# aikiriao/LINNE

Hardware: AMD Instinct MI355X
Metric: frames/sec encode (-m 7) + decode, 44.1 kHz stereo, bit-exact; 1/2/4/8 GPU (higher is better)
Workload: dtype f64; 1 GPU; encode -m 7: 1 x 60 min 44.1 kHz int16 2-channel per GPU = 15504 frames of 10240 samples (tail 9280), MS on, PCM resident in HBM; decode = inverse hot path on the encode output; frames_per_gpu=15504, channels=2, preset=7, tracks_per_gpu=1

## Files before the change

linne_amd/csrc/lnn_k_autocorr.h:

```cpp
#ifndef LNN_K_AUTOCORR_H_INCLUDED
#define LNN_K_AUTOCORR_H_INCLUDED

__device__ __forceinline__ const DevClass &job_class(const Plan &p, uint32_t job) { return p.cls[p.cls_of_frame[(job / p.R) / p.C]]; }
__device__ __forceinline__ double q1_stale_first_trial(const Plan &p, uint32_t job, const DevClass &c)
{
    const uint32_t f = (job / p.R) / p.C, mid = c.na >> 1;
    if (mid >= c.n) return 0.0;
    const size_t i = ((size_t)p.frame_map[f] * p.C + (p.C - 1u)) * p.S + mid;
    return ((double)pcm_at(p, i) * p.scale) * p.sintab[c.sin_off + mid];
}

template <int P> struct AcCfg {
    static constexpr int K = 5;
    static constexpr int NT = (P >= 128) ? 8 : ((P >= 64) ? 7 : (P >= 32) ? 6 : (P >= 16) ? 5 : (P >= 8) ? 4 : (P >= 4) ? 3 : 2);
    static constexpr int T = (P >= 32) ? 60 : 20;
    static constexpr int lanes(int t) { return ((P >> t) + 1 + K - 1) / K; }
    static constexpr int halo(int t) { return K * lanes(t) + K; }
    static constexpr int rb(int t) { return ((T + halo(t) + 3 + 4 * K - 1) / (4 * K)) * (4 * K); }
    static constexpr int lpj() { int s = 0; for (int t = 0; t < NT; t++) s += lanes(t); return s; }
    static constexpr int ringsum() { int s = 0; for (int t = 0; t < NT; t++) s += rb(t); return s; }
    static constexpr int maxpad() { int m = 0; for (int t = 0; t < NT; t++) { const int p = P >> t, z = p > 4 ? p : 4, v = (1 << t) * z; if (v > m) m = v; } return m; }
    static constexpr int LPJ = lpj();
    static constexpr int JPW = 64 / LPJ;
    static constexpr int NS = JPW * NT;
// ... 239 lines not shown
__device__ __forceinline__ void autocorr_lane(const Plan &p, uint32_t layer, uint32_t cur, uint32_t q_end, uint32_t job, uint32_t t, bool active)
{
    constexpr int U = 4;
    constexpr uint32_t np = K - 1;
    const DevClass &c = job_class(p, job);
    const uint32_t u = 1u << t;
    const uint32_t n = active ? (c.na / u) : 1u;
    const uint32_t upl = n + (np > 4 ? np : 4);
    const double *wt = p.wtab + (active ? c.wt_off[layer][t] : 0u);
    const int32_t *xi = p.xint + (size_t)(job / p.R) * p.S;
    const double *xd = p.sig + ((size_t)job * 2 + cur) * p.S;
    double stale = 0.0;
    if (active && (n & 1u) && u == 1u) stale = q1_stale_first_trial(p, job, c);
    else if (active && (n & 1u)) {
        const uint32_t m = n >> 1, n2 = 2 * n, si = (u / 2 - 1) * n2 + m;
        const double xv = L0 ? ((double)xi[si] * p.scale) : xd[si];
        stale = xv * (c.trial_div[layer][t - 1] * (double)m * (double)(n2 - 1 - m));
    }
    const bool odd = (n & 1u) != 0;
    const uint32_t mid = n >> 1;
    uint32_t g_loc = 0, g_ubase = 0, g_left = active ? u : 0u;
    auto gen_issue = [&](double &rx, double &rw, uint32_t &rloc) {
        const bool in_unit = (g_loc < n) && (g_left != 0);
        rx = L0 ? ((double)xi[in_unit ? (g_ubase + g_loc) : 0u] * p.scale) : xd[in_unit ? (g_ubase + g_loc) : 0u];
        rw = wt[g_loc];
        rloc = in_unit ? g_loc : 0xFFFFFFFFu;
        const bool wrap = (g_loc + 1 >= upl);
        g_loc = wrap ? 0u : g_loc + 1;
        g_ubase = (wrap && g_left > 1) ? g_ubase + n : g_ubase;
        g_left = (wrap && g_left) ? g_left - 1 : g_left;
    };
    auto gen_finish = [&](double rx, double rw, uint32_t rloc) -> double {
        const double v = rx * rw;
        const double vv = (odd && rloc == mid) ? stale : v;
        return (rloc == 0xFFFFFFFFu) ? 0.0 : vv;
    };
    double r[K], w[K + U], fx[D][U], fw[D][U]; uint32_t fl[D][U];
#pragma unroll
    for (int j = 0; j < K; j++) {
        r[j] = 0.0;
        double rx, rw; uint32_t rl;
        gen_issue(rx, rw, rl);
        w[j] = gen_finish(rx, rw, rl);
    }
#pragma unroll
    for (int d = 0; d < D; d++) {
#pragma unroll
        for (int j = 0; j < U; j++) gen_issue(fx[d][j], fw[d][j], fl[d][j]);
    }
    uint32_t a_unit = 0, flush_pos = n;
    double *out = p.acorr + ((size_t)job * LNN_MAXT + t) * LNN_ACW;
#pragma unroll 1
    for (uint32_t q0 = 0; q0 < q_end; q0 += U * D) {
#pragma unroll
        for (int d = 0; d < D; d++) {
            if (active && q0 + (uint32_t)(d * U) >= flush_pos) {
                double *o = out + (size_t)a_unit * K;
#pragma unroll
                for (int j = 0; j < K; j++) { o[j] = r[j]; r[j] = 0.0; }
                a_unit++;
                flush_pos = (a_unit < u) ? (flush_pos + upl) : 0xFFFFFFFFu;
            }
#pragma unroll
            for (int j = 0; j < U; j++) w[K + j] = gen_finish(fx[d][j], fw[d][j], fl[d][j]);
#pragma unroll
            for (int j = 0; j < U; j++) gen_issue(fx[d][j], fw[d][j], fl[d][j]);
#pragma unroll
            for (int tt = 0; tt < U; tt++) {
#pragma unroll
                for (int j = 0; j < K; j++) r[j] += w[tt] * w[tt + j];
            }
#pragma unroll
            for (int j = 0; j < K; j++) w[j] = w[j + U];
        }
    }
}

#define ACS_T 32
template <int K, int J0, int JN, bool L0, int NT>
__device__ __forceinline__ void autocorr_shared(const Plan &p, uint32_t layer, uint32_t cur, uint32_t row0, uint32_t nrows, uint32_t rstride,
        uint32_t na, uint32_t wt_off, uint32_t t, uint32_t wave, uint32_t lane, double (*tile)[ACS_T][65])
{
    constexpr uint32_t np = K - 1, pad = (np > 4 ? np : 4);
    constexpr int L = ((int)np + 3) / 4 * 4;
    constexpr int NSLOT = (ACS_T + NT - 1) / NT;
    const uint32_t u = 1u << t, n = na / u, upl = n + pad, ntiles = na / ACS_T;
    const double *wt = p.wtab + wt_off;
    uint32_t myrow = row0 + lane; if (myrow >= nrows) myrow = nrows - 1;
    const bool store = (row0 + lane) < nrows;
    double *out = p.acorr + ((size_t)myrow * rstride * LNN_MAXT + t) * LNN_ACW;
    double preA[NSLOT], preB[NSLOT], wA = 0.0, wB = 0.0, wcur = 0.0;
    const uint32_t ls = lane & (ACS_T - 1u), lr = lane / ACS_T;
    constexpr uint32_t RPS = 64 / ACS_T;
    auto issue = [&](uint32_t tile_idx, double *pre, double &wv) {
#pragma unroll
        for (int i = 0; i < NSLOT; i++) {
            const uint32_t k = wave + (uint32_t)i * NT;
            if (k < 64 / RPS) {
                uint32_t r = row0 + RPS * k + lr; if (r >= nrows) r = nrows - 1;
                const uint32_t sidx = tile_idx * ACS_T + ls;
                if (L0) pre[i] = (double)p.xint[(size_t)r * p.S + sidx] * p.scale;
                else pre[i] = p.sig[((size_t)r * 2 + cur) * p.S + sidx];
            }
        }
        wv = wt[(tile_idx * ACS_T + ls) % n];
    };
    auto commit = [&](uint32_t buf, const double *pre, double wv) {
#pragma unroll
        for (int i = 0; i < NSLOT; i++) {
            const uint32_t k = wave + (uint32_t)i * NT;
            if (k < 64 / RPS) tile[buf][ls][RPS * k + lr] = pre[i];
        }
        wcur = wv;
    };
    auto lane_bcast = [&](double v, uint32_t src_lane) -> double {
        const int lo = __builtin_amdgcn_readlane(__double2loint(v), (int)src_lane), hi = __builtin_amdgcn_readlane(__double2hiint(v), (int)src_lane);
        return __hiloint2double(hi, lo);
    };
    issue(0, preA, wA); commit(0, preA, wA);
    __syncthreads();
    if (ntiles > 1) issue(1, preB, wB);
    if (ntiles > 2) issue(2, preA, wA);
    uint32_t g_loc = 0, g_tile = 0, g_off = 0;
    struct D4 { double v0, v1, v2, v3; };
    auto next4 = [&]() -> D4 {
        D4 d; d.v0 = 0.0; d.v1 = 0.0; d.v2 = 0.0; d.v3 = 0.0;
        if (g_loc < n && g_tile < ntiles) {
            const double *src = &tile[g_tile & 1u][g_off][lane];
            d.v0 = src[0] * lane_bcast(wcur, g_off); d.v1 = src[65] * lane_bcast(wcur, g_off + 1);
            d.v2 = src[130] * lane_bcast(wcur, g_off + 2); d.v3 = src[195] * lane_bcast(wcur, g_off + 3);
            g_off += 4;
            if (g_off == ACS_T) {
                g_off = 0; g_tile++;
                if (g_tile < ntiles) {
                    if (g_tile & 1u) { commit(1, preB, wB); __syncthreads(); if (g_tile + 2 < ntiles) issue(g_tile + 2, preB, wB); }
                    else             { commit(0, preA, wA); __syncthreads(); if (g_tile + 2 < ntiles) issue(g_tile + 2, preA, wA); }
                }
            }
        }
        g_loc += 4; if (g_loc >= upl) g_loc = 0;
        return d;
    };
    constexpr int W = L + 4, NG = W / 4;
    double r[JN], w[W];
#pragma unroll
    for (int j = 0; j < JN; j++) r[j] = 0.0;
#pragma unroll
    for (int j = 0; j < L / 4; j++) { const D4 d = next4(); w[4 * j] = d.v0; w[4 * j + 1] = d.v1; w[4 * j + 2] = d.v2; w[4 * j + 3] = d.v3; }
    uint32_t a_unit = 0, flush_pos = n, q0 = 0;
    bool done = false;
#pragma unroll 1
    while (!done) {
#pragma unroll
        for (int g = 0; g < NG; g++) {
            if (!done) {
                if (q0 >= flush_pos) {
                    if (store) {
                        double *o = out + (size_t)a_unit * K + J0;
#pragma unroll
                        for (int j = 0; j < JN; j++) o[j] = r[j];
                    }
#pragma unroll
                    for (int j = 0; j < JN; j++) r[j] = 0.0;
                    a_unit++;
                    flush_pos += upl;
                    done = (a_unit == u);
                }
                if (!done) {
                    const D4 d = next4();
                    w[(4 * g + L) % W] = d.v0; w[(4 * g + L + 1) % W] = d.v1; w[(4 * g + L + 2) % W] = d.v2; w[(4 * g + L + 3) % W] = d.v3;
#pragma unroll
                    for (int tt = 0; tt < 4; tt++) {
#pragma unroll
                        for (int j = 0; j < JN; j++) r[j] += w[(4 * g + tt) % W] * w[(4 * g + tt + J0 + j) % W];
                    }
                    q0 += 4;
                }
            }
        }
    }
}

template <int P, bool L0, int TT, int J0, int JN, int NW, int T = 32>
__device__ __forceinline__ void autocorr_rows(const Plan &p, uint32_t layer, uint32_t cur, uint32_t row0, uint32_t nrows, uint32_t rstride,
        uint32_t na, const DevClass &c0, uint32_t wave, uint32_t lane, double (*xt)[T][65], double (*wtile)[32])
{
    constexpr int NT = AcCfg<P>::NT, NLD = L0 ? T / 4 : T / 2, PT = P >> TT;
    constexpr int NSLOT = (NLD + NW - 1) / NW;
    constexpr int TU = (PT > T) ? PT / T : 1;
    constexpr uint32_t RPI = L0 ? 256u / T : 128u / T, LPR = 64u / RPI;
    static_assert((T == 32 || T == 16) && PT <= 32 && (TU * T) % PT == 0 && J0 + JN <= PT + 1, "register rings: sample m lives in slot m % PT, and the tile loop is unrolled over TU * T samples");
    typedef typename std::conditional<L0, int4, lnn_d2>::type XV;
    const uint32_t ntiles = na / T, seg = na >> (NT - 1), nt = na >> TT;
    uint32_t myrow = row0 + lane; if (myrow >= nrows) myrow = nrows - 1;
    const bool store = (row0 + lane) < nrows;
    double *out = p.acorr + ((size_t)myrow * rstride * LNN_MAXT + TT) * LNN_ACW + J0;
    const uint32_t lrow = lane / LPR, lsmp = (L0 ? 4u : 2u) * (lane % LPR);
    const void *src[NSLOT];
#pragma unroll
    for (int i = 0; i < NSLOT; i++) {
        const uint32_t k = wave + (uint32_t)i * NW;
        uint32_t r = row0 + RPI * (k < (uint32_t)NLD ? k : 0u) + lrow; if (r >= nrows) r = nrows - 1;
        if (L0) src[i] = p.xint + (size_t)r * p.S + lsmp;
        else src[i] = p.sig + ((size_t)r * 2 + cur) * p.S + lsmp;
    }
    const double *wt = p.wtab + (uint32_t)__builtin_amdgcn_readfirstlane((int)c0.wt_off[layer][TT]);
    const double *wts = p.wtab + (uint32_t)__builtin_amdgcn_readfirstlane((int)c0.wt_off[layer][wave < (uint32_t)NT ? wave : 0u]);
    const uint32_t wnt = na >> (wave < (uint32_t)NT ? wave : 0u);
    uint32_t wloc = 0;
    (void)wt; (void)nt;
    XV pre[NSLOT]; double prew = 0.0;
    auto issue = [&](uint32_t tile_idx) {
#pragma unroll
        for (int i = 0; i < NSLOT; i++)
            if (wave + (uint32_t)i * NW < (uint32_t)NLD) pre[i] = *(const XV *)((L0 ? (const char *)src[i] + (size_t)tile_idx * T * 4 : (const char *)src[i] + (size_t)tile_idx * T * 8));
        if (wave < (uint32_t)NT) {
            uint32_t l = wloc + (lane & (T - 1u)); if (l >= wnt) l -= wnt;
            prew = wts[l];
            wloc += T; if (wloc >= wnt) wloc -= wnt;
        }
    };
    auto commit = [&](uint32_t buf) {
#pragma unroll
        for (int i = 0; i < NSLOT; i++) {
            const uint32_t k = wave + (uint32_t)i * NW;
            if (k < (uint32_t)NLD) {
                const uint32_t r = RPI * k + lrow;
                if (L0) {
                    const int4 v = *(const int4 *)&pre[i];
                    xt[buf][lsmp][r] = (double)v.x * p.scale; xt[buf][lsmp + 1][r] = (double)v.y * p.scale;
                    xt[buf][lsmp + 2][r] = (double)v.z * p.scale; xt[buf][lsmp + 3][r] = (double)v.w * p.scale;
                } else { const lnn_d2 v = *(const lnn_d2 *)&pre[i]; xt[buf][lsmp][r] = v.x; xt[buf][lsmp + 1][r] = v.y; }
            }
        }
        if (wave < (uint32_t)NT && lane < T) wtile[buf * NT + wave][lane] = prew;
    };
    double r[JN], ring[PT], q[JN];
#pragma unroll
    for (int j = 0; j < JN; j++) { r[j] = 0.0; q[j] = 0.0; }
#pragma unroll
    for (int j = 0; j < PT; j++) ring[j] = 0.0;
    auto read_group = [&](uint32_t slot, double *xv, double *wv) {
        const uint32_t buf = slot / T, o = slot % T;
#pragma unroll
        for (int i = 0; i < 4; i++) xv[i] = xt[buf][o + i][lane];
        const lnn_d2 a = *(const lnn_d2 *)&wtile[buf * NT + TT][o], b = *(const lnn_d2 *)&wtile[buf * NT + TT][o + 2];
        wv[0] = a.x; wv[1] = a.y; wv[2] = b.x; wv[3] = b.y;
    };
    issue(0); commit(0);
    __syncthreads();
    double xv[4], wv[4], vcur;
    read_group(0, xv, wv);
    vcur = xv[0] * wv[0];
    uint32_t to_b = seg, bcount = 0, unit = 0;
#pragma unroll 1
    for (uint32_t t0 = 0; t0 < ntiles; t0 += TU) {
#pragma unroll
      for (int h = 0; h < TU; h++) {
        const uint32_t ti = t0 + (uint32_t)h, buf = ti & 1u;
        if (ti + 1 < ntiles) issue(ti + 1);
#pragma unroll
        for (int g = 0; g < T / 4; g++) {
            if (g == T / 4 - 1) {
                if (ti + 1 < ntiles) commit(buf ^ 1u);
                __syncthreads();
            }
            double nx[4], nw[4];
            read_group((buf * T + 4 * (uint32_t)g + 4) % (2 * T), nx, nw);
#pragma unroll
            for (int i = 0; i < 4; i++) {
#pragma unroll
                for (int j = 0; j < JN; j++) r[j] += q[j];
                const double v = vcur;
#pragma unroll
                for (int j = 0; j < JN; j++) q[j] = (J0 + j == 0) ? (v * v) : (ring[((h * T + 4 * g + i - (J0 + j)) % PT + PT) % PT] * v);
                ring[(h * T + 4 * g + i) % PT] = v;
                vcur = (i < 3) ? (xv[(i + 1) & 3] * wv[(i + 1) & 3]) : (nx[0] * nw[0]);
            }
#pragma unroll
            for (int i = 0; i < 4; i++) { xv[i] = nx[i]; wv[i] = nw[i]; }
            to_b -= 4;
            if (to_b == 0) {
                to_b = seg; bcount++;
                if ((bcount & ((1u << (NT - 1 - TT)) - 1u)) == 0) {
#pragma unroll
                    for (int j = 0; j < JN; j++) { r[j] += q[j]; q[j] = 0.0; }
                    if (store) {
                        double *o = out + (size_t)unit * (PT + 1);
#pragma unroll
                        for (int j = 0; j < JN; j++) o[j] = r[j];
                    }
#pragma unroll
                    for (int j = 0; j < JN; j++) r[j] = 0.0;
#pragma unroll
                    for (int j = 0; j < PT; j++) ring[j] = 0.0;
                    unit++;
                }
            }
        }
      }
    }
}

template <int P> struct AcsWaves;
template <> struct AcsWaves<16> { static constexpr int NW = 8; };
template <> struct AcsWaves<8>  { static constexpr int NW = 5; };
template <> struct AcsWaves<4>  { static constexpr int NW = 10; };
template <> struct AcsWaves<2>  { static constexpr int NW = 5; };

#define ACS_ROWS(P_) ((P_) <= 4 || p.rows16)
template <int P, bool L0>
__global__ __launch_bounds__(64 * AcsWaves<P>::NW, (P >= 8) ? 4 : 5) void k_autocorr_lane(Plan p, uint32_t layer, uint32_t cur, uint32_t na_max)
{
    using Cfg = AcCfg<P>;
    constexpr int NT = Cfg::NT, NW = AcsWaves<P>::NW;
    __shared__ double tile[2][ACS_T][65];
    __shared__ __attribute__((aligned(16))) double wts_mem[2 * NT * 32];
    const uint32_t wave = threadIdx.x >> 6, lane = threadIdx.x & 63u;
    const uint32_t rstride = L0 ? p.R : 1u;
    const RowRuns &rr = p.runs[L0 ? 0 : 1];
    const uint32_t b = gridDim.x - 1u - blockIdx.x;
    uint32_t run = 0;
    while (run + 1 < rr.n && b >= rr.blk_begin[run + 1]) run++;
    const uint32_t row0 = rr.row_begin[run] + (b - rr.blk_begin[run]) * 64u, nrows = rr.row_begin[run + 1];
    uint32_t row = row0 + lane;
    const bool inrange = row < nrows;
    if (!inrange) row = nrows - 1;
    const uint32_t job = row * rstride;
    const uint32_t ci = p.cls_of_frame[(job / p.R) / p.C];
    const uint32_t ci0 = (uint32_t)__builtin_amdgcn_readfirstlane((int)ci);
    const DevClass &c0 = p.cls[ci0];
    const uint32_t na = (uint32_t)__builtin_amdgcn_readfirstlane((int)c0.na);
    const bool fast = __all(ci == ci0) && c0.ntrials[layer] == (uint32_t)NT && (na % (4u << (NT - 1))) == 0 && (na % ACS_T) == 0;
    constexpr int NWS = (P == 4) ? 3 : (P == 2) ? 2 : NW;
#define ACS_RUN(T_, K_, J0_, JN_) autocorr_shared<K_, J0_, JN_, L0, NWS>(p, layer, cur, row0, nrows, rstride, na, \
        (uint32_t)__builtin_amdgcn_readfirstlane((int)c0.wt_off[layer][T_]), T_, wave, lane, tile)
    if constexpr (P <= 16) {
        if (fast && (na >> (NT - 1)) >= 32u && (p.S & 3u) == 0 && ACS_ROWS(P)) {
            double (*wtile)[32] = (double (*)[32])wts_mem;
#define ROWS_RUN(T_, J0_, JN_) autocorr_rows<P, L0, T_, J0_, JN_, NW>(p, layer, cur, row0, nrows, rstride, na, c0, wave, lane, tile, wtile)
            if constexpr (P == 16) switch (wave) {
                case 0: ROWS_RUN(0, 10, 7); break; case 1: ROWS_RUN(0, 0, 5); break; case 2: ROWS_RUN(0, 5, 5); break; case 3: ROWS_RUN(1, 0, 5); break;
                case 4: ROWS_RUN(4, 0, 2); break;  case 5: ROWS_RUN(1, 5, 4); break; case 6: ROWS_RUN(2, 0, 5); break; default: ROWS_RUN(3, 0, 3); break;
            } else if constexpr (P == 8) switch (wave) {
                case 0: ROWS_RUN(0, 0, 5); break; case 1: ROWS_RUN(0, 5, 4); break; case 2: ROWS_RUN(1, 0, 5); break; case 3: ROWS_RUN(2, 0, 3); break;
                default: ROWS_RUN(3, 0, 2); break;
            } else if constexpr (P == 4) switch (wave) {
                case 0: ROWS_RUN(0, 0, 1); break; case 1: ROWS_RUN(0, 1, 1); break; case 2: ROWS_RUN(0, 2, 1); break; case 3: ROWS_RUN(0, 3, 1); break;
                case 4: ROWS_RUN(0, 4, 1); break; case 5: ROWS_RUN(1, 0, 1); break; case 6: ROWS_RUN(1, 1, 1); break; case 7: ROWS_RUN(1, 2, 1); break;
                case 8: ROWS_RUN(2, 0, 1); break; default: ROWS_RUN(2, 1, 1); break;
            } else switch (wave) {
                case 0: ROWS_RUN(0, 0, 1); break; case 1: ROWS_RUN(0, 1, 1); break; case 2: ROWS_RUN(0, 2, 1); break;
                case 3: ROWS_RUN(1, 0, 1); break; default: ROWS_RUN(1, 1, 1); break;
            }
#undef ROWS_RUN
            return;
        }
    }
    if (fast) {
        if (P == 16) switch (wave) {
            case 0: ACS_RUN(0, 17, 10, 7); break; case 1: ACS_RUN(0, 17, 0, 5); break;  case 2: ACS_RUN(0, 17, 5, 5); break;
            case 3: ACS_RUN(1, 9, 0, 5); break;   case 4: ACS_RUN(4, 2, 0, 2); break;   case 5: ACS_RUN(1, 9, 5, 4); break;
            case 6: ACS_RUN(2, 5, 0, 5); break;   default: ACS_RUN(3, 3, 0, 3); break;
        } else if (P == 8) switch (wave) {
            case 0: ACS_RUN(0, 9, 0, 5); break;   case 1: ACS_RUN(0, 9, 5, 4); break;   case 2: ACS_RUN(1, 5, 0, 5); break;
            case 3: ACS_RUN(2, 3, 0, 3); break;   default: ACS_RUN(3, 2, 0, 2); break;
        } else if (P == 4) switch (wave) {
            case 0: ACS_RUN(0, 5, 0, 5); break;   case 1: ACS_RUN(1, 3, 0, 3); break;   case 2: ACS_RUN(2, 2, 0, 2); break;   default: break;
        } else switch (wave) {
            case 0: ACS_RUN(0, 3, 0, 3); break;   case 1: ACS_RUN(1, 2, 0, 2); break;   default: break;
        }
        return;
    }
#undef ACS_RUN
    if (wave >= (uint32_t)NT) return;
    const uint32_t t = wave;
    const bool active = inrange && (t < job_class(p, job).ntrials[layer]);
    constexpr int D = 1;
    const uint32_t q_end = na_max + Cfg::MAXPAD + 8 + 4 * D;
    switch (P >> t) {
    case 16: if (P >= 16) autocorr_lane<17, L0, D>(p, layer, cur, q_end, job, t, active); break;
    case 8:  if (P >= 8)  autocorr_lane<9, L0, D>(p, layer, cur, q_end, job, t, active); break;
    case 4:  if (P >= 4)  autocorr_lane<5, L0, D>(p, layer, cur, q_end, job, t, active); break;
    case 2:  autocorr_lane<3, L0, D>(p, layer, cur, q_end, job, t, active); break;
    default: autocorr_lane<2, L0, D>(p, layer, cur, q_end, job, t, active); break;
    }
}

template <int P> static void launch_autocorr_small(hipStream_t st, const Plan &p, uint32_t layer, uint32_t cur, uint32_t na_max)
{
    const RowRuns &rr = p.runs[layer == 0 ? 0 : 1];
    const dim3 grid(rr.blk_begin[rr.n]);
    if (layer == 0) hipLaunchKernelGGL((k_autocorr_lane<P, true>), grid, dim3(64 * AcsWaves<P>::NW), 0, st, p, layer, cur, na_max);
    else hipLaunchKernelGGL((k_autocorr_lane<P, false>), grid, dim3(64 * AcsWaves<P>::NW), 0, st, p, layer, cur, na_max);
}

template <int P> struct ApCfg {
    static constexpr int NT = (P >= 16) ? 5 : (P >= 8) ? 4 : (P >= 4) ? 3 : 2;
    static constexpr int nch() { int s = 0; for (int t = 0; t < NT; t++) s += (P >> t) + 1; return s; }
    static constexpr int NCH = nch();
    static constexpr int CHUNK = (P >= 16) ? 128 : (P >= 8) ? 128 : 256;
    static constexpr int trial_of(int ch) { int t = 0; while (ch >= (P >> t) + 1) { ch -= (P >> t) + 1; t++; } return t; }
    static constexpr int lag_of(int ch) { int t = 0; while (ch >= (P >> t) + 1) { ch -= (P >> t) + 1; t++; } return ch; }
};
template <int P, bool L0, int NTH>
__global__ __launch_bounds__(NTH) void k_autocorr_prod(Plan p, uint32_t layer, uint32_t cur)
{
    using Cfg = ApCfg<P>;
    constexpr int NT = Cfg::NT, NCH = Cfg::NCH, CHUNK = Cfg::CHUNK, NPROD = NTH - 64;
    static_assert(NCH <= 64, "one wave adds up all chains");
    __shared__ double sv[2][NT][CHUNK + P];
    __shared__ uint32_t srem[2][NT][CHUNK + P];
    __shared__ __attribute__((aligned(16))) double sprod[2][NCH][CHUNK + 2];
    const uint32_t row = blockIdx.x, tid = threadIdx.x, job = L0 ? row * p.R : row;
    const DevClass &c = job_class(p, job);
    const uint32_t na = c.na;
    const int32_t *xi = p.xint + (size_t)(job / p.R) * p.S;
    const double *xd = p.sig + ((size_t)job * 2 + cur) * p.S;
    const uint32_t nchunks = (na + CHUNK - 1) / CHUNK;
    const bool producer = tid >= 64u;
    const uint32_t ptid = tid - 64u;
    uint32_t ct = 0, clag = tid;
    while (ct + 1 < (uint32_t)NT && clag >= ((uint32_t)P >> ct) + 1) { clag -= ((uint32_t)P >> ct) + 1; ct++; }
    const uint32_t cn = na >> ct, cnp = (uint32_t)P >> ct;
    double r = 0.0;
    uint32_t cloc = 0, cunit = 0;
    double *cout = p.acorr + ((size_t)job * LNN_MAXT + ct) * LNN_ACW + clag;
    constexpr int NPRE = (CHUNK + P + NPROD - 1) / NPROD;
    double px[NPRE], pw[NPRE][NT];
    uint32_t wloc[NPRE][NT], prem[NPRE][NT];
#pragma unroll
    for (int m = 0; m < NPRE; m++)
#pragma unroll
        for (int t = 0; t < NT; t++) wloc[m][t] = (ptid + (uint32_t)m * NPROD) % (na >> t);
    auto prefetch = [&](uint32_t kk) {
        const uint32_t base = kk * CHUNK;
#pragma unroll
        for (int m = 0; m < NPRE; m++) {
            const uint32_t i = ptid + (uint32_t)m * NPROD, g = base + i;
            const bool in = i < (uint32_t)(CHUNK + P) && g < na;
            px[m] = in ? (L0 ? ((double)xi[g] * p.scale) : xd[g]) : 0.0;
#pragma unroll
            for (int t = 0; t < NT; t++) {
                const uint32_t nt = na >> t;
                pw[m][t] = in ? p.wtab[c.wt_off[layer][t] + wloc[m][t]] : 0.0;
                prem[m][t] = nt - 1u - wloc[m][t];
                uint32_t l = wloc[m][t] + (uint32_t)CHUNK;
                while (l >= nt) l -= nt;
                wloc[m][t] = l;
            }
        }
    };
    constexpr int NPM = (NCH * CHUNK + NPROD - 1) / NPROD;
    uint32_t pe[NPM];
#pragma unroll
    for (int m = 0; m < NPM; m++) {
        const uint32_t e = ptid + (uint32_t)m * NPROD, ch = e / (uint32_t)CHUNK, i = e % (uint32_t)CHUNK;
        uint32_t t = 0, lag = ch;
        while (t + 1 < (uint32_t)NT && lag >= ((uint32_t)P >> t) + 1) { lag -= ((uint32_t)P >> t) + 1; t++; }
        pe[m] = (ch < (uint32_t)NCH) ? (i | (ch << 12) | (lag << 20) | (t << 28)) : 0xFFFFFFFFu;
    }
    if (producer) prefetch(0);
    for (uint32_t k = 0; k < nchunks + 2u; k++) {
        if (producer) {
            if (k < nchunks) {
                double (*dst)[CHUNK + P] = sv[k & 1u];
                uint32_t (*drem)[CHUNK + P] = srem[k & 1u];
#pragma unroll
                for (int m = 0; m < NPRE; m++) {
                    const uint32_t i = ptid + (uint32_t)m * NPROD;
                    if (i < (uint32_t)(CHUNK + P)) {
#pragma unroll
                        for (int t = 0; t < NT; t++) { dst[t][i] = px[m] * pw[m][t]; drem[t][i] = prem[m][t]; }
                    }
                }
                if (k + 1u < nchunks && !LNN_DBG_IS(p, 103u)) prefetch(k + 1u);
            }
            if (k >= 1u && k - 1u < nchunks && !LNN_DBG_IS(p, 102u)) {
                const double (*src)[CHUNK + P] = sv[(k - 1u) & 1u];
                const uint32_t (*rem)[CHUNK + P] = srem[(k - 1u) & 1u];
                double (*dst)[CHUNK + 2] = sprod[(k - 1u) & 1u];
                double av[NPM], bv[NPM]; uint32_t rv[NPM];
#pragma unroll
                for (int m = 0; m < NPM; m++) {
                    const uint32_t e = (pe[m] != 0xFFFFFFFFu) ? pe[m] : 0u;
                    const uint32_t i = e & 0xFFFu, lag = (e >> 20) & 0xFFu, t = e >> 28;
                    av[m] = src[t][i]; bv[m] = src[t][i + lag]; rv[m] = rem[t][i];
                }
#pragma unroll
                for (int m = 0; m < NPM; m++) {
                    const uint32_t e = pe[m];
                    if (e != 0xFFFFFFFFu) {
                        const uint32_t i = e & 0xFFFu, ch = (e >> 12) & 0xFFu, lag = (e >> 20) & 0xFFu;
                        dst[ch][i] = (lag <= rv[m]) ? av[m] * bv[m] : 0.0;
                    }
                }
            }
        } else if (k >= 2u && tid < (uint32_t)NCH && !LNN_DBG_IS(p, 101u)) {
            const uint32_t base = (k - 2u) * CHUNK;
            const uint32_t cnt = (na - base < (uint32_t)CHUNK) ? (na - base) : (uint32_t)CHUNK;
            const double *q = sprod[k & 1u][tid];
            uint32_t i = 0;
            while (i < cnt) {
                const uint32_t seg = (cnt - i < cn - cloc) ? (cnt - i) : (cn - cloc), end = i + seg;
#define AP_LOAD(A, OFF) { const lnn_d2 *q2_ = (const lnn_d2 *)(q + i + (OFF)); A##0 = q2_[0]; A##1 = q2_[1]; A##2 = q2_[2]; A##3 = q2_[3]; }
#define AP_ADD(A) { r += (A##0).x; r += (A##0).y; r += (A##1).x; r += (A##1).y; r += (A##2).x; r += (A##2).y; r += (A##3).x; r += (A##3).y; }
                if (i + 16 <= end) {
                    lnn_d2 a0, a1, a2, a3, b0, b1, b2, b3;
                    AP_LOAD(a, 0)
                    for (; i + 16 <= end; i += 16) {
                        AP_LOAD(b, 8)
                        AP_ADD(a)
                        if (i + 24 <= end) AP_LOAD(a, 16)
                        AP_ADD(b)
                    }
                }
                if (i + 8 <= end) { lnn_d2 a0, a1, a2, a3; AP_LOAD(a, 0) AP_ADD(a) i += 8; }
#undef AP_LOAD
#undef AP_ADD
                for (; i < end; i++) r += q[i];
                cloc += seg;
                if (cloc == cn) { cout[(size_t)cunit * (cnp + 1)] = r; r = 0.0; cloc = 0; cunit++; }
            }
        }
        __syncthreads();
    }
}

template <int P> static void launch_autocorr2(hipStream_t st, const Plan &p, uint32_t layer, uint32_t cur, uint32_t na_max)
{
    using Cfg = AcCfg<P>;
    const uint32_t blocks = (p.J + Cfg::JPW - 1) / Cfg::JPW;
    if (layer == 0) hipLaunchKernelGGL((k_autocorr2<P, true>), dim3(blocks), dim3(64), 0, st, p, layer, cur, na_max);
    else hipLaunchKernelGGL((k_autocorr2<P, false>), dim3(blocks), dim3(64), 0, st, p, layer, cur, na_max);
}
#include "lnn_k_autocorr_hist.h"

static bool launch_autocorr_hist(hipStream_t st, const Plan &p, uint32_t layer, uint32_t cur, int which, bool small_sub = false)
{
    const RowRuns &rr = p.runs[1];
    const dim3 grid(rr.blk_begin[rr.n]);
    if (p.P[layer] == 128u) {
        if (which == 0) hipLaunchKernelGGL((k_autocorr_hist<128, 0>), grid, dim3(64 * HIST_WAVES(128)), 0, st, p, layer, cur);
        else if (which == 1) hipLaunchKernelGGL((k_autocorr_hist<128, 1>), grid, dim3(64 * HIST_WAVES(64)), 0, st, p, layer, cur);
        else if (small_sub) hipLaunchKernelGGL((k_autocorr_sub<128, LNN_SUB_TILE_SMALL>), grid, dim3(640), 0, st, p, layer, cur);
        else hipLaunchKernelGGL((k_autocorr_sub<128>), grid, dim3(640), 0, st, p, layer, cur);
        return true;
    }
    if (p.P[layer] == 64u) {
        if (which == 0) hipLaunchKernelGGL((k_autocorr_hist<64, 0>), grid, dim3(64 * HIST_WAVES(64)), 0, st, p, layer, cur);
        else if (which == 2) hipLaunchKernelGGL((k_autocorr_sub<64>), grid, dim3(640), 0, st, p, layer, cur);
        else return false;
        return true;
    }
    return false;
}

#define AW_TILE 512
template <int P>
__global__ __launch_bounds__(64 * ((P + 64) / 64)) void k_autocorr_wide(Plan p, uint32_t layer, uint32_t cur)
{
    constexpr int NTHR = 64 * ((P + 64) / 64);
    constexpr int NPRE = (AW_TILE + P + NTHR - 1) / NTHR;
    __shared__ __attribute__((aligned(16))) double xs[AW_TILE + P + 8];
    const uint32_t row = blockIdx.x, t = blockIdx.y, tid = threadIdx.x;
    const bool l0 = (layer == 0);
    const uint32_t job = l0 ? row * p.R : row;
    const DevClass &c = job_class(p, job);
    if (t >= c.ntrials[layer]) return;
    const uint32_t na = c.na, u = 1u << t, np = (uint32_t)P >> t, nt = na >> t;
    const int32_t *xi = p.xint + (size_t)(job / p.R) * p.S;
    const double *xd = p.sig + ((size_t)job * 2 + cur) * p.S;
    const double *wt = p.wtab + c.wt_off[layer][t];
    double *out = p.acorr + ((size_t)job * LNN_MAXT + t) * LNN_ACW + tid;
    const bool mine = tid <= np;
    const uint32_t tiles_per_unit = (nt + AW_TILE - 1) / AW_TILE, ntiles = u * tiles_per_unit;
    double px[NPRE], pwv[NPRE];
    auto prefetch = [&](uint32_t ti) {
        const uint32_t un = ti / tiles_per_unit, loc0 = (ti - un * tiles_per_unit) * AW_TILE;
#pragma unroll
        for (int m = 0; m < NPRE; m++) {
            const uint32_t i = tid + (uint32_t)m * NTHR, loc = loc0 + i;
            const bool in = i < (uint32_t)AW_TILE + np && loc < nt;
            const uint32_t g = un * nt + loc;
            px[m] = in ? (l0 ? ((double)xi[g] * p.scale) : xd[g]) : 0.0;
            pwv[m] = in ? wt[loc] : 0.0;
        }
    };
    prefetch(0);
    double acc = 0.0;
    for (uint32_t ti = 0; ti < ntiles; ti++) {
        const uint32_t un = ti / tiles_per_unit, loc0 = (ti - un * tiles_per_unit) * AW_TILE;
        __syncthreads();
#pragma unroll
        for (int m = 0; m < NPRE; m++) { const uint32_t i = tid + (uint32_t)m * NTHR; if (i < (uint32_t)AW_TILE + np) xs[i] = px[m] * pwv[m]; }
        if (ti + 1 < ntiles) prefetch(ti + 1);
        __syncthreads();
        if (mine) {
            const uint32_t cnt = (nt - loc0 < (uint32_t)AW_TILE) ? (nt - loc0) : (uint32_t)AW_TILE;
            const double *xa = xs, *xb = xs + tid;
            uint32_t j = 0;
            for (; j + 32 <= cnt; j += 32) {
                double m[32];
#pragma unroll
                for (int q = 0; q < 32; q += 2) { const lnn_d2 a = *(const lnn_d2 *)(xa + j + q); m[q] = a.x * xb[j + q]; m[q + 1] = a.y * xb[j + q + 1]; }
#pragma unroll
                for (int q = 0; q < 32; q++) acc += m[q];
            }
            for (; j + 16 <= cnt; j += 16) {
                double m[16];
#pragma unroll
                for (int q = 0; q < 16; q += 2) { const lnn_d2 a = *(const lnn_d2 *)(xa + j + q); m[q] = a.x * xb[j + q]; m[q + 1] = a.y * xb[j + q + 1]; }
#pragma unroll
                for (int q = 0; q < 16; q++) acc += m[q];
            }
            for (; j + 8 <= cnt; j += 8) {
                const lnn_d2 a0 = *(const lnn_d2 *)(xa + j), a1 = *(const lnn_d2 *)(xa + j + 2), a2 = *(const lnn_d2 *)(xa + j + 4), a3 = *(const lnn_d2 *)(xa + j + 6);
                const double b0 = xb[j], b1 = xb[j + 1], b2 = xb[j + 2], b3 = xb[j + 3], b4 = xb[j + 4], b5 = xb[j + 5], b6 = xb[j + 6], b7 = xb[j + 7];
                const double m0 = a0.x * b0, m1 = a0.y * b1, m2 = a1.x * b2, m3 = a1.y * b3, m4 = a2.x * b4, m5 = a2.y * b5, m6 = a3.x * b6, m7 = a3.y * b7;
                acc += m0; acc += m1; acc += m2; acc += m3; acc += m4; acc += m5; acc += m6; acc += m7;
            }
            for (; j < cnt; j++) acc += xa[j] * xb[j];
            if (loc0 + cnt == nt) { out[(size_t)un * (np + 1)] = acc; acc = 0.0; }
        }
    }
}

static void dispatch_autocorr2(hipStream_t st, const Plan &p, uint32_t layer, uint32_t cur, uint32_t na_max, bool prod_ok)
{
    if (prod_ok && p.P[layer] <= 16u) {
        const uint32_t rows = (layer == 0) ? p.J / p.R : p.J;
        const bool small = (layer == 0) ? (rows < 6144u) : (rows <= 512u);
        if (small) {
#define LNN_AP(PP, NTH_) do { if (layer == 0) hipLaunchKernelGGL((k_autocorr_prod<PP, true, NTH_>), dim3(rows), dim3(NTH_), 0, st, p, layer, cur); \
                        else hipLaunchKernelGGL((k_autocorr_prod<PP, false, NTH_>), dim3(rows), dim3(NTH_), 0, st, p, layer, cur); } while (0)
            switch (p.P[layer]) { case 2: LNN_AP(2, 256); break; case 4: LNN_AP(4, 256); break; case 8: LNN_AP(8, 512); break; default: LNN_AP(16, 512); break; }
#undef LNN_AP
            return;
        }
    }
    if (prod_ok && p.P[layer] >= 32u) {
        const uint32_t rows = (layer == 0) ? p.J / p.R : p.J;
        uint32_t ntr = 0; for (uint32_t u = 1; u <= (p.P[layer] < (uint32_t)LNN_MAXU ? p.P[layer] : (uint32_t)LNN_MAXU); u <<= 1) ntr++;
        switch (p.P[layer]) {
        case 32: hipLaunchKernelGGL((k_autocorr_wide<32>), dim3(rows, ntr), dim3(64), 0, st, p, layer, cur); break;
        case 64: hipLaunchKernelGGL((k_autocorr_wide<64>), dim3(rows, ntr), dim3(128), 0, st, p, layer, cur); break;
        default: hipLaunchKernelGGL((k_autocorr_wide<128>), dim3(rows, ntr), dim3(192), 0, st, p, layer, cur); break;
        }
        return;
    }
    switch (p.P[layer]) {
    case 2: launch_autocorr_small<2>(st, p, layer, cur, na_max); break;
    case 4: launch_autocorr_small<4>(st, p, layer, cur, na_max); break;
    case 8: launch_autocorr_small<8>(st, p, layer, cur, na_max); break;
    case 16: launch_autocorr_small<16>(st, p, layer, cur, na_max); break;
    case 32: launch_autocorr2<32>(st, p, layer, cur, na_max); break;
    case 64: launch_autocorr2<64>(st, p, layer, cur, na_max); break;
    default: launch_autocorr2<128>(st, p, layer, cur, na_max); break;
    }
}


#endif
```

linne_amd/csrc/lnn_k_autocorr_hist.h:

```cpp
#ifndef LNN_K_AUTOCORR_HIST_H_INCLUDED
#define LNN_K_AUTOCORR_HIST_H_INCLUDED

__device__ __forceinline__ void lds_dma16(const void *g, void *lds_wave_base)
{
    const uint32_t base = (uint32_t)(size_t)(__attribute__((address_space(3))) void *)lds_wave_base;
    uint32_t keep;
    asm volatile("s_mov_b32 %0, m0\n\ts_mov_b32 m0, %1\n\ts_nop 0\n\tglobal_load_lds_dwordx4 %2, off\n\ts_mov_b32 m0, %0" : "=&s"(keep) : "s"(base), "v"(g) : "memory");
}
#define HIST_ACC(i_) "+v"(r[i_])
template <int N> __device__ __forceinline__ void hist_wait_loads(double (&r)[N])
{
    static_assert(N == 2 || N == 8 || N == 9 || N == 11, "one operand list per lag count");
    if constexpr (N == 2)
        asm volatile("s_waitcnt vmcnt(0)" : HIST_ACC(0), HIST_ACC(1) : : "memory");
    else if constexpr (N == 8)
        asm volatile("s_waitcnt vmcnt(0)" : HIST_ACC(0), HIST_ACC(1), HIST_ACC(2), HIST_ACC(3), HIST_ACC(4), HIST_ACC(5), HIST_ACC(6), HIST_ACC(7) : : "memory");
    else if constexpr (N == 9)
        asm volatile("s_waitcnt vmcnt(0)" : HIST_ACC(0), HIST_ACC(1), HIST_ACC(2), HIST_ACC(3), HIST_ACC(4), HIST_ACC(5), HIST_ACC(6), HIST_ACC(7), HIST_ACC(8) : : "memory");
    else
        asm volatile("s_waitcnt vmcnt(0)" : HIST_ACC(0), HIST_ACC(1), HIST_ACC(2), HIST_ACC(3), HIST_ACC(4), HIST_ACC(5), HIST_ACC(6), HIST_ACC(7), HIST_ACC(8), HIST_ACC(9), HIST_ACC(10) : : "memory");
}
#undef HIST_ACC
#define HIST_LPW(PT_) ((PT_) >= 128 ? 11 : 9)
#define HIST_TILE(PT_) 16
#define HIST_WAVES(PT_) (((PT_) + HIST_LPW(PT_)) / HIST_LPW(PT_))
template <int P, int TT>
__global__ __launch_bounds__(64 * HIST_WAVES(P >> TT), ((P >> TT) >= 128) ? 3 : 4) void k_autocorr_hist(Plan p, uint32_t layer, uint32_t cur)
{
    constexpr int PT = P >> TT, NLAG = PT + 1, LPW = HIST_LPW(PT), NW = HIST_WAVES(PT), NLAST = NLAG - LPW * (NW - 1), T = HIST_TILE(PT), D = PT + 2 * T, NLD = T / 2, RPI = 128 / T;
    constexpr int NSLOT = (NLD + NW - 1) / NW;
    static_assert(LPW <= 16, "a wave's lags come from a 16-deep register ring");
    static_assert(NLAST >= 1 && NLAST <= LPW, "the last wave takes the lags the full waves leave");
    static_assert(PT % T == 0 && D % T == 0, "tiles must not straddle a unit's end or the ring's end");
    __shared__ __attribute__((aligned(16))) double ring_lds[D + T][65];
    __shared__ __attribute__((aligned(16))) lnn_d2 stage[NLD][64];
    const uint32_t wave = (uint32_t)__builtin_amdgcn_readfirstlane((int)(threadIdx.x >> 6)), lane = threadIdx.x & 63u;
    const RowRuns &rr = p.runs[1];
    const uint32_t b = gridDim.x - 1u - blockIdx.x;
    uint32_t run = 0;
    while (run + 1 < rr.n && b >= rr.blk_begin[run + 1]) run++;
    const uint32_t row0 = rr.row_begin[run] + (b - rr.blk_begin[run]) * 64u, nrows = rr.row_begin[run + 1];
    uint32_t myrow = row0 + lane; if (myrow >= nrows) myrow = nrows - 1;
    const bool store = (row0 + lane) < nrows;
    const uint32_t ci = p.cls_of_frame[(myrow / p.R) / p.C];
    const uint32_t ci0 = (uint32_t)__builtin_amdgcn_readfirstlane((int)ci);
    const DevClass &c0 = p.cls[ci0];
    if (!__all(ci == ci0) || !hist_takes(p, layer, c0)) return;
    const uint32_t na = (uint32_t)__builtin_amdgcn_readfirstlane((int)c0.na);
    const uint32_t n = na >> TT, upl = n + (uint32_t)PT, units = 1u << TT, total = units * upl, ntiles = total / T;
    const double *wt = p.wtab + (uint32_t)__builtin_amdgcn_readfirstlane((int)c0.wt_off[layer][TT]);
    const uint32_t J0 = wave * (uint32_t)LPW;
    double *out = p.acorr + ((size_t)myrow * LNN_MAXT + TT) * LNN_ACW + J0;
    for (uint32_t i = threadIdx.x; i < (uint32_t)(D + T) * 65u; i += blockDim.x) (&ring_lds[0][0])[i] = 0.0;
    const uint32_t lrow = lane / (uint32_t)(T / 2), lsmp = 2u * (lane % (uint32_t)(T / 2));
    const double *src[NSLOT];
#pragma unroll
    for (int i = 0; i < NSLOT; i++) {
        const uint32_t k = wave + (uint32_t)i * NW;
        uint32_t lr = row0 + (uint32_t)RPI * (k < (uint32_t)NLD ? k : 0u) + lrow; if (lr >= nrows) lr = nrows - 1;
        src[i] = p.sig + ((size_t)lr * 2 + cur) * p.S + lsmp;
    }
    uint32_t f_unit = 0, f_loc = 0;
    uint32_t p_loc = 0;
    const double wdiv = c0.trial_div[layer][TT];
    (void)wt;
    auto issue = [&]() {
        p_loc = f_loc;
#pragma unroll
        for (int i = 0; i < NSLOT; i++) {
            const uint32_t k = wave + (uint32_t)i * NW;
            if (k < (uint32_t)NLD && f_loc < n)
                lds_dma16(src[i] + (size_t)f_unit * n + f_loc, &stage[k][0]);
        }
        f_loc += T; if (f_loc == upl) { f_loc = 0; f_unit++; }
    };
    auto welch = [&](uint32_t loc) -> double {
        const uint32_t h = (loc < (n >> 1)) ? loc : (n - 1u - loc);
        return wdiv * (double)h * (double)(n - 1u - h);
    };
    auto lags = [&](auto nj) __attribute__((always_inline)) {
    constexpr int NJ = decltype(nj)::value;
    double r[NJ], q[NJ], hist[16];
#pragma unroll
    for (int j = 0; j < NJ; j++) { r[j] = 0.0; q[j] = 0.0; }
#pragma unroll
    for (int j = 0; j < 16; j++) hist[j] = 0.0;
    auto commit = [&](uint32_t slot0) {
        hist_wait_loads(r);
#pragma unroll
        for (int i = 0; i < NSLOT; i++) {
            const uint32_t k = wave + (uint32_t)i * NW;
            if (k < (uint32_t)NLD) {
                const uint32_t r = (uint32_t)RPI * k + lrow;
                double vx = 0.0, vy = 0.0;
                if (p_loc < n) { const lnn_d2 x = stage[k][lane]; vx = x.x * welch(p_loc + lsmp); vy = x.y * welch(p_loc + lsmp + 1u); }
                ring_lds[slot0 + lsmp][r] = vx; ring_lds[slot0 + lsmp + 1][r] = vy;
                if (slot0 == 0) { ring_lds[D + lsmp][r] = vx; ring_lds[D + lsmp + 1][r] = vy; }
            }
        }
    };
    __syncthreads();
    issue(); commit(0);
    __syncthreads();
    uint32_t slot_c = 0, slot_d = (uint32_t)((D - (int)(J0 % (uint32_t)D)) % D);
    auto read_group = [&](uint32_t sc, uint32_t sd, double *cv, double *dv) {
#pragma unroll
        for (int i = 0; i < 4; i++) { cv[i] = ring_lds[sc + i][lane]; dv[i] = ring_lds[sd + i][lane]; }
    };
    double cv[4], dv[4];
    read_group(slot_c, slot_d, cv, dv);
    uint32_t a_unit = 0, a_loc = 0;
#pragma unroll 1
    for (uint32_t ti = 0; ti < ntiles; ti++) {
        if (ti + 1 < ntiles) issue();
#pragma unroll
        for (int g = 0; g < T / 4; g++) {
            double ncv[4], ndv[4];
            if (g == T / 4 - 1) {
                uint32_t nslot = slot_c + T; if (nslot == (uint32_t)D) nslot = 0;
                if (ti + 1 < ntiles) commit(nslot);
                __syncthreads();
                uint32_t nd = slot_d + T; if (nd >= (uint32_t)D) nd -= (uint32_t)D;
                read_group(nslot, nd, ncv, ndv);
                slot_c = nslot; slot_d = nd;
            } else read_group(slot_c + 4 * (g + 1), slot_d + 4 * (g + 1), ncv, ndv);
#pragma unroll
            for (int i = 0; i < 4; i++) {
#pragma unroll
                for (int j = 0; j < NJ; j++) r[j] += q[j];
                hist[(4 * g + i) % 16] = dv[i];
                const double v = cv[i];
#pragma unroll
                for (int j = 0; j < NJ; j++) q[j] = hist[((4 * g + i - j) % 16 + 16) % 16] * v;
            }
#pragma unroll
            for (int i = 0; i < 4; i++) { cv[i] = ncv[i]; dv[i] = ndv[i]; }
        }
        a_loc += T;
        if (a_loc == upl) {
#pragma unroll
            for (int j = 0; j < NJ; j++) { r[j] += q[j]; q[j] = 0.0; }
            if (store) {
                double *o = out + (size_t)a_unit * NLAG;
#pragma unroll
                for (int j = 0; j < NJ; j++) o[j] = r[j];
            }
#pragma unroll
            for (int j = 0; j < NJ; j++) r[j] = 0.0;
            a_loc = 0; a_unit++;
        }
    }
    };
    if (wave == (uint32_t)(NW - 1)) lags(std::integral_constant<int, NLAST>{});
    else lags(std::integral_constant<int, LPW>{});
}

template <int P, int T = 32>
__global__ __launch_bounds__(640, 3) void k_autocorr_sub(Plan p, uint32_t layer, uint32_t cur)
{
    constexpr int NT = AcCfg<P>::NT, NW = 10, T0 = NT - 6;
    __shared__ double tile[2][T][65];
    __shared__ __attribute__((aligned(16))) double wts_mem[2 * NT * 32];
    static_assert(T == 32 || sizeof(double) * (2 * T * 65 + 2 * NT * 32) <= LNN_SUB_SMALL_LDS, "lnn_forms.h counts on the small form's LDS");
    static_assert((16 << (NT - 1)) % (2 * T) == 0, "hist_takes must imply an even number of tiles");
    const uint32_t wave = threadIdx.x >> 6, lane = threadIdx.x & 63u;
    const RowRuns &rr = p.runs[1];
    const uint32_t b = gridDim.x - 1u - blockIdx.x;
    uint32_t run = 0;
    while (run + 1 < rr.n && b >= rr.blk_begin[run + 1]) run++;
    const uint32_t row0 = rr.row_begin[run] + (b - rr.blk_begin[run]) * 64u, nrows = rr.row_begin[run + 1];
    uint32_t row = row0 + lane; if (row >= nrows) row = nrows - 1;
    const uint32_t ci = p.cls_of_frame[(row / p.R) / p.C];
    const uint32_t ci0 = (uint32_t)__builtin_amdgcn_readfirstlane((int)ci);
    const DevClass &c0 = p.cls[ci0];
    if (!__all(ci == ci0) || !hist_takes(p, layer, c0)) return;
    const uint32_t na = (uint32_t)__builtin_amdgcn_readfirstlane((int)c0.na);
    double (*wtile)[32] = (double (*)[32])wts_mem;
#define SUB_RUN(T_, J0_, JN_) autocorr_rows<P, false, T_, J0_, JN_, NW, T>(p, layer, cur, row0, nrows, 1u, na, c0, wave, lane, tile, wtile)
    switch (wave) {
        case 0: SUB_RUN(T0, 0, 9); break;      case 1: SUB_RUN(T0, 9, 8); break;      case 2: SUB_RUN(T0, 17, 8); break;   case 3: SUB_RUN(T0, 25, 8); break;
        case 4: SUB_RUN(T0 + 1, 0, 9); break;  case 5: SUB_RUN(T0 + 1, 9, 8); break;  case 6: SUB_RUN(T0 + 2, 0, 9); break;
        case 7: SUB_RUN(T0 + 3, 0, 5); break;  case 8: SUB_RUN(T0 + 4, 0, 3); break;  default: SUB_RUN(T0 + 5, 0, 2); break;
    }
#undef SUB_RUN
}

#endif
```

Before: 222,100 frames/s.

## Rebalance autocorr sub kernel into eight waves with checked lag-role tables

Replaces the hand-written per-wave switch statements with constexpr lag-role tables that are checked at compile time to cover every lag exactly once. For the P=16 lane kernel the roles stay the same. The order-32..1 sub kernel drops from ten waves to eight, with wider lag slices per wave (11/11/11, then 17 for the next trial). The aim is less per-block overhead and better tile reuse per wave, at the cost of more registers per wave and a longer critical path on the widest wave.

```diff
diff --git a/linne_amd/csrc/lnn_k_autocorr.h b/linne_amd/csrc/lnn_k_autocorr.h
--- a/linne_amd/csrc/lnn_k_autocorr.h
+++ b/linne_amd/csrc/lnn_k_autocorr.h
@@ -565,8 +565,39 @@
     }
 }
 
+struct LagRole { int t, j0, jn; };
+template <int N> constexpr int lag_role_count(const LagRole (&)[N]) { return N; }
+template <int N> constexpr bool lag_roles_ok(const LagRole (&r)[N], int P, int t_first, int t_last)
+{
+    for (int i = 0; i < N; i++)
+        if (r[i].t < t_first || r[i].t > t_last || r[i].j0 < 0 || r[i].jn < 1 || r[i].j0 + r[i].jn > (P >> r[i].t) + 1) return false;
+    for (int t = t_first; t <= t_last; t++) {
+        uint64_t owned = 0; int sum = 0;
+        for (int i = 0; i < N; i++) {
+            if (r[i].t != t) continue;
+            const uint64_t m = (((uint64_t)1 << r[i].jn) - 1u) << r[i].j0;
+            if (owned & m) return false;
+            owned |= m; sum += r[i].jn;
+        }
+        if (sum != (P >> t) + 1 || owned != ((uint64_t)1 << ((P >> t) + 1)) - 1u) return false;
+    }
+    return true;
+}
+template <int N, int W = 0, class F> __device__ __forceinline__ void lag_role_of_wave(uint32_t wave, F &&f)
+{
+    if constexpr (W + 1 >= N) f(std::integral_constant<int, N - 1>{});
+    else if (wave == (uint32_t)W) f(std::integral_constant<int, W>{});
+    else lag_role_of_wave<N, W + 1>(wave, f);
+}
+
+struct AcsRoles16 {
+    static constexpr LagRole roles[] = { {0, 10, 7}, {0, 0, 5}, {0, 5, 5}, {1, 0, 5}, {4, 0, 2}, {1, 5, 4}, {2, 0, 5}, {3, 0, 3} };
+    static constexpr int NW = lag_role_count(roles);
+    static_assert(lag_roles_ok(roles, 16, 0, AcCfg<16>::NT - 1), "every lag of every trial has exactly one wave");
+    static_assert(NW >= AcCfg<16>::NT, "the first NT waves fetch the trials' weights (autocorr_rows) and take a trial each in the general form");
+};
 template <int P> struct AcsWaves;
-template <> struct AcsWaves<16> { static constexpr int NW = 8; };
+template <> struct AcsWaves<16> { static constexpr int NW = AcsRoles16::NW; };
 template <> struct AcsWaves<8>  { static constexpr int NW = 5; };
 template <> struct AcsWaves<4>  { static constexpr int NW = 10; };
 template <> struct AcsWaves<2>  { static constexpr int NW = 5; };
@@ -602,10 +633,11 @@
         if (fast && (na >> (NT - 1)) >= 32u && (p.S & 3u) == 0 && ACS_ROWS(P)) {
             double (*wtile)[32] = (double (*)[32])wts_mem;
 #define ROWS_RUN(T_, J0_, JN_) autocorr_rows<P, L0, T_, J0_, JN_, NW>(p, layer, cur, row0, nrows, rstride, na, c0, wave, lane, tile, wtile)
-            if constexpr (P == 16) switch (wave) {
-                case 0: ROWS_RUN(0, 10, 7); break; case 1: ROWS_RUN(0, 0, 5); break; case 2: ROWS_RUN(0, 5, 5); break; case 3: ROWS_RUN(1, 0, 5); break;
-                case 4: ROWS_RUN(4, 0, 2); break;  case 5: ROWS_RUN(1, 5, 4); break; case 6: ROWS_RUN(2, 0, 5); break; default: ROWS_RUN(3, 0, 3); break;
-            } else if constexpr (P == 8) switch (wave) {
+            if constexpr (P == 16) lag_role_of_wave<NW>(wave, [&](auto w) __attribute__((always_inline)) {
+                constexpr LagRole R = AcsRoles16::roles[decltype(w)::value];
+                ROWS_RUN(R.t, R.j0, R.jn);
+            });
+            else if constexpr (P == 8) switch (wave) {
                 case 0: ROWS_RUN(0, 0, 5); break; case 1: ROWS_RUN(0, 5, 4); break; case 2: ROWS_RUN(1, 0, 5); break; case 3: ROWS_RUN(2, 0, 3); break;
                 default: ROWS_RUN(3, 0, 2); break;
             } else if constexpr (P == 4) switch (wave) {
@@ -621,11 +653,11 @@
         }
     }
     if (fast) {
-        if (P == 16) switch (wave) {
-            case 0: ACS_RUN(0, 17, 10, 7); break; case 1: ACS_RUN(0, 17, 0, 5); break;  case 2: ACS_RUN(0, 17, 5, 5); break;
-            case 3: ACS_RUN(1, 9, 0, 5); break;   case 4: ACS_RUN(4, 2, 0, 2); break;   case 5: ACS_RUN(1, 9, 5, 4); break;
-            case 6: ACS_RUN(2, 5, 0, 5); break;   default: ACS_RUN(3, 3, 0, 3); break;
-        } else if (P == 8) switch (wave) {
+        if constexpr (P == 16) lag_role_of_wave<NW>(wave, [&](auto w) __attribute__((always_inline)) {
+            constexpr LagRole R = AcsRoles16::roles[decltype(w)::value];
+            ACS_RUN((uint32_t)R.t, (16 >> R.t) + 1, R.j0, R.jn);
+        });
+        else if (P == 8) switch (wave) {
             case 0: ACS_RUN(0, 9, 0, 5); break;   case 1: ACS_RUN(0, 9, 5, 4); break;   case 2: ACS_RUN(1, 5, 0, 5); break;
             case 3: ACS_RUN(2, 3, 0, 3); break;   default: ACS_RUN(3, 2, 0, 2); break;
         } else if (P == 4) switch (wave) {
@@ -806,13 +838,13 @@
     if (p.P[layer] == 128u) {
         if (which == 0) hipLaunchKernelGGL((k_autocorr_hist<128, 0>), grid, dim3(64 * HIST_WAVES(128)), 0, st, p, layer, cur);
         else if (which == 1) hipLaunchKernelGGL((k_autocorr_hist<128, 1>), grid, dim3(64 * HIST_WAVES(64)), 0, st, p, layer, cur);
-        else if (small_sub) hipLaunchKernelGGL((k_autocorr_sub<128, LNN_SUB_TILE_SMALL>), grid, dim3(640), 0, st, p, layer, cur);
-        else hipLaunchKernelGGL((k_autocorr_sub<128>), grid, dim3(640), 0, st, p, layer, cur);
+        else if (small_sub) hipLaunchKernelGGL((k_autocorr_sub<128, LNN_SUB_TILE_SMALL>), grid, dim3(64 * SubRoles<128>::NW), 0, st, p, layer, cur);
+        else hipLaunchKernelGGL((k_autocorr_sub<128>), grid, dim3(64 * SubRoles<128>::NW), 0, st, p, layer, cur);
         return true;
     }
     if (p.P[layer] == 64u) {
         if (which == 0) hipLaunchKernelGGL((k_autocorr_hist<64, 0>), grid, dim3(64 * HIST_WAVES(64)), 0, st, p, layer, cur);
-        else if (which == 2) hipLaunchKernelGGL((k_autocorr_sub<64>), grid, dim3(640), 0, st, p, layer, cur);
+        else if (which == 2) hipLaunchKernelGGL((k_autocorr_sub<64>), grid, dim3(64 * SubRoles<64>::NW), 0, st, p, layer, cur);
         else return false;
         return true;
     }
diff --git a/linne_amd/csrc/lnn_k_autocorr_hist.h b/linne_amd/csrc/lnn_k_autocorr_hist.h
--- a/linne_amd/csrc/lnn_k_autocorr_hist.h
+++ b/linne_amd/csrc/lnn_k_autocorr_hist.h
@@ -155,10 +155,17 @@
     else lags(std::integral_constant<int, LPW>{});
 }
 
+template <int P> struct SubRoles {
+    static constexpr int T0 = AcCfg<P>::NT - 6;
+    static constexpr LagRole roles[] = { {T0, 0, 11}, {T0, 11, 11}, {T0, 22, 11}, {T0 + 1, 0, 17}, {T0 + 2, 0, 9}, {T0 + 3, 0, 5}, {T0 + 4, 0, 3}, {T0 + 5, 0, 2} };
+    static constexpr int NW = lag_role_count(roles);
+    static_assert(lag_roles_ok(roles, P, T0, AcCfg<P>::NT - 1), "every lag of the trials of order 32 .. 1 has exactly one wave");
+    static_assert(NW >= AcCfg<P>::NT, "the block's first NT waves fetch the trials' weights (autocorr_rows)");
+};
 template <int P, int T = 32>
-__global__ __launch_bounds__(640, 3) void k_autocorr_sub(Plan p, uint32_t layer, uint32_t cur)
+__global__ __launch_bounds__(64 * SubRoles<P>::NW, 3) void k_autocorr_sub(Plan p, uint32_t layer, uint32_t cur)
 {
-    constexpr int NT = AcCfg<P>::NT, NW = 10, T0 = NT - 6;
+    constexpr int NT = AcCfg<P>::NT, NW = SubRoles<P>::NW;
     __shared__ double tile[2][T][65];
     __shared__ __attribute__((aligned(16))) double wts_mem[2 * NT * 32];
     static_assert(T == 32 || sizeof(double) * (2 * T * 65 + 2 * NT * 32) <= LNN_SUB_SMALL_LDS, "lnn_forms.h counts on the small form's LDS");
@@ -176,13 +183,10 @@
     if (!__all(ci == ci0) || !hist_takes(p, layer, c0)) return;
     const uint32_t na = (uint32_t)__builtin_amdgcn_readfirstlane((int)c0.na);
     double (*wtile)[32] = (double (*)[32])wts_mem;
-#define SUB_RUN(T_, J0_, JN_) autocorr_rows<P, false, T_, J0_, JN_, NW, T>(p, layer, cur, row0, nrows, 1u, na, c0, wave, lane, tile, wtile)
-    switch (wave) {
-        case 0: SUB_RUN(T0, 0, 9); break;      case 1: SUB_RUN(T0, 9, 8); break;      case 2: SUB_RUN(T0, 17, 8); break;   case 3: SUB_RUN(T0, 25, 8); break;
-        case 4: SUB_RUN(T0 + 1, 0, 9); break;  case 5: SUB_RUN(T0 + 1, 9, 8); break;  case 6: SUB_RUN(T0 + 2, 0, 9); break;
-        case 7: SUB_RUN(T0 + 3, 0, 5); break;  case 8: SUB_RUN(T0 + 4, 0, 3); break;  default: SUB_RUN(T0 + 5, 0, 2); break;
-    }
-#undef SUB_RUN
+    lag_role_of_wave<NW>(wave, [&](auto w) __attribute__((always_inline)) {
+        constexpr LagRole R = SubRoles<P>::roles[decltype(w)::value];
+        autocorr_rows<P, false, R.t, R.j0, R.jn, NW, T>(p, layer, cur, row0, nrows, 1u, na, c0, wave, lane, tile, wtile);
+    });
 }
 
 #endif
```

Result: no change. 220,700 frames/s (-0.6%).
